# ducha-aiki/mods-light-zmq

Hardware: AMD Instinct MI355X
Metric: image_pairs_per_sec_end_to_end (higher is better)
Workload: dtype f32

## Files before the change

### include/mods_hip.h

```cpp
#ifndef MODS_HIP_H
#define MODS_HIP_H

#include <stddef.h>
#include <stdint.h>

#ifdef __cplusplus
extern "C" {
#endif

#define MODS_OK 0
#define MODS_E_NODEVICE (-1)
#define MODS_E_ARG (-2)
#define MODS_E_CAPACITY (-3)
#define MODS_E_HIP (-4)

typedef struct mods_ctx mods_ctx;

typedef struct mods_hessaff_params {
  int numberOfScales;
  float initialSigma;
  float threshold;
  float edgeEigenValueRatio;
  int border;
  int maxIterations;
// ... 68 lines not shown
       MODS_STAGE_LOCAL_AFFINE,
       MODS_STAGE_COUNT };
int mods_ctx_timing_enable(mods_ctx *ctx, int stage_mask);
int mods_ctx_graphs(mods_ctx *ctx, int on);
long mods_ctx_graph_replays(const mods_ctx *ctx);
long mods_ctx_u8_source_calls(const mods_ctx *ctx);
int mods_ctx_u8_kernels(mods_ctx *ctx, int mask);
long mods_ctx_u8_strip_calls(const mods_ctx *ctx);
int mods_u8_strips_layout(int w, int h, unsigned *max_width, unsigned *n_strips, unsigned *pitch, size_t *image_bytes);
void mods_u8_strips_strip_of(unsigned n, unsigned *out);
int mods_u8_strips_offsets(int w, int h, unsigned *out);
int mods_u8_strips_fetch(mods_ctx *ctx, const unsigned char *img_u8_host, int n_img, int w, int h, int src_offset, unsigned char *out);
int mods_ctx_pyramid_streams(mods_ctx *ctx, int n);
int mods_ctx_timing_read(mods_ctx *ctx, int stage, double *total_ms, int *launches, double *bytes);
int mods_ctx_timing_reset(mods_ctx *ctx);

int mods_detect_hessian_affine(mods_ctx *ctx, const float *img, int w, int h, int stride,
                               const mods_hessaff_params *par, mods_affkey *out, int max_out, int *n_out);
int mods_detect_hessian_affine_dev(mods_ctx *ctx, const float *img_dev, int n_img, int w, int h, int stride,
                                   const mods_hessaff_params *par, mods_affkey *out_host, int max_out,
                                   int *n_out_host);

int mods_pyramid_octaves(mods_ctx *ctx);
int mods_pyramid_dims(mods_ctx *ctx, int octave, int *w, int *h);
int mods_pyramid_plane(mods_ctx *ctx, int img, int octave, int level, int kind, float *dst_host);
int mods_pyramid_candidates(mods_ctx *ctx, int img, mods_candidate *out, int max_out, int *n_out);
int mods_pyramid_nms_hits(mods_ctx *ctx, int img, int *out4, int max_out, int *n_out);

int mods_gauss_blur(mods_ctx *ctx, const float *src, int w, int h, float sigma, float *dst);
int mods_hessian_response(mods_ctx *ctx, const float *src, int w, int h, float norm, float *dst);
int mods_resize_half(mods_ctx *ctx, const float *src, int w, int h, float *dst, int *dw, int *dh);

typedef struct mods_describe_params {
  double ori_mrSize;
  int ori_patchSize;
  int ori_maxAngles;
  double ori_threshold;
  double desc_mrSize;
  int desc_patchSize;
  int photoNorm;
  int rootSift;
  double maxBinValue;
  int ori_halfMode;
  int addUpRight;
  int halfDesc;
  int fastExtraction;
} mods_describe_params;

int mods_orient_describe(mods_ctx *ctx, const float *img, int w, int h, int stride, const mods_affkey *keys,
                         int n_keys, const mods_describe_params *par, mods_region *out, int max_out, int *n_out);

int mods_orient_describe_u8(mods_ctx *ctx, const unsigned char *img_u8, int w, int h, int stride, const mods_affkey *keys,
                            int n_keys, const mods_describe_params *par, mods_region *out, int max_out, int *n_out);

int mods_detect_describe_dev(mods_ctx *ctx, const float *img_dev, int n_img, int w, int h, int stride,
                             const mods_hessaff_params *det, const mods_describe_params *desc,
                             int *n_detected_host, int *n_regions_host);
int mods_detect_describe_dev_u8(mods_ctx *ctx, const unsigned char *img_u8_dev, int n_img, int w, int h, int stride,
                                const mods_hessaff_params *det, const mods_describe_params *desc,
                                int *n_detected_host, int *n_regions_host);
typedef int (*mods_descriptor_fn)(void *user, const float *patches, int n, int ps, float *out, size_t out_cap_floats, int *dim);
int mods_ctx_set_external_descriptor(mods_ctx *ctx, mods_descriptor_fn fn, void *user, double mrSize, int patchSize);
int mods_ctx_set_external_shape(mods_ctx *ctx, mods_descriptor_fn fn, void *user, double mrSize, int patchSize);
int mods_ctx_set_external_orientation(mods_ctx *ctx, mods_descriptor_fn fn, void *user, double mrSize, int patchSize);
typedef struct mods_net mods_net;
enum { MODS_NET_AFFNET = 0, MODS_NET_ORINET = 1, MODS_NET_HARDNET = 2 };
int  mods_net_create(int device, int kind, const float *const *tensors, const size_t *n_floats, int n_tensors, mods_net **out);
void mods_net_destroy(mods_net *net);
int  mods_net_dim(const mods_net *net);
int  mods_net_chunk(void);
int  mods_net_forward(mods_net *net, const float *patches_host, int n, int quantise_u8, float *out_host);
int  mods_net_forward_dev(mods_net *net, void *hip_stream, const float *patches_dev, int n, int quantise_u8, float *out_dev);
int  mods_ctx_set_builtin_shape(mods_ctx *ctx, mods_net *net, double mrSize, int quantise_u8);
int  mods_ctx_set_builtin_orientation(mods_ctx *ctx, mods_net *net, double mrSize, int quantise_u8);
int  mods_ctx_set_builtin_descriptor(mods_ctx *ctx, mods_net *net, double mrSize, int quantise_u8);
int  mods_test_net_stage(mods_net *net, int stage, const float *in_host, int n, int quantise_u8, float *out_host, int *guard_ok);
int mods_patches_fetch(mods_ctx *ctx, int img, int ps, float *out, int max_regions, int *n_out);
int mods_baumberg_stats_enable(mods_ctx *ctx, int on);
int mods_baumberg_stats(mods_ctx *ctx, int img, unsigned long long *keypoints, unsigned long long *iterations);
int mods_unoriented_count(mods_ctx *ctx, int img);
int mods_regions_fetch(mods_ctx *ctx, int img, mods_region *out, int max_out, int *n_out);

int mods_dominant_angle(mods_ctx *ctx, const float *patch, int ps, double th, float *angle, int *found);
int mods_selftest_fast_sqrt(mods_ctx *ctx, unsigned long long *out5);
int mods_sift_patch(mods_ctx *ctx, const float *patch, int ps, int rootsift, double maxBinValue, uint8_t *out128);

typedef struct mods_view_geom {
  int identity;
  int w_rot, h_rot;
  int w_new, h_new;
  int ksize_x, ksize_y, pad;
  double rotation, tilt, zoom;
  double sigma_x, sigma_y;
  double H[9];
  double warpRot[6], warpTilt[6];
} mods_view_geom;

int mods_view_geometry(int w, int h, double tilt, double phi, double zoom, double initSigma, mods_view_geom *out);
int mods_synth_view_dev(mods_ctx *ctx, const float *src_dev, int w, int h, int stride, const mods_view_geom *geom, int doBlur,
                        float *dst_dev);
int mods_detect_describe_view_dev(mods_ctx *ctx, const float *src_dev, int w, int h, int stride, double tilt, double phi,
                                  double zoom, double initSigma, int doBlur, const mods_hessaff_params *det,
                                  const mods_describe_params *desc, mods_view_geom *geom_out, int *n_detected, int *n_regions);
int mods_detect_describe_view2_dev(mods_ctx *ctx, const float *src1_dev, const float *src2_dev, int w, int h, int stride, double tilt,
                                   double phi, double zoom, double initSigma, int doBlur, const mods_hessaff_params *det,
                                   const mods_describe_params *desc, mods_view_geom *geom_out, int *n_detected2, int *n_regions2);
const mods_region *mods_regions_dev(mods_ctx *ctx, int img);
const mods_region *mods_regions_half_dev(mods_ctx *ctx, int img);
int mods_regions_fetch_half(mods_ctx *ctx, int img, mods_region *out, int max_out, int *n_out);
int mods_regions_copy_dev(mods_ctx *ctx, int img, mods_region *dst_dev, int n);
const float *mods_view_pixels_dev(mods_ctx *ctx);
int mods_view_fetch(mods_ctx *ctx, const mods_view_geom *geom, float *dst_host);
int mods_warp_affine(mods_ctx *ctx, const float *src, int w, int h, const double *M, int dw, int dh, float cval, float *dst);
int mods_gauss_blur_xy(mods_ctx *ctx, const float *src, int w, int h, int kx, int ky, double sx, double sy, float *dst);

int mods_match_fginn(mods_ctx *ctx, const mods_region *q, int n_q, const mods_region *t, int n_t, double ratio,
                     double contradDist, int nn, mods_tentative *out, double *u6_out, double *laf_out, int max_out, int *n_out);
int mods_match_distance(mods_ctx *ctx, const mods_region *q, int n_q, const mods_region *t, int n_t, double threshold,
                        mods_tentative *out, double *u6_out, double *laf_out, int max_out, int *n_out);
int mods_match_dev(mods_ctx *ctx, int img_q, int img_t, double ratio, double contradDist, int nn, mods_tentative *out,
                   double *u6_out, double *laf_out, int max_out, int *n_out);
int mods_match_grid(int n_q, int n_t, int out[3]);

int mods_duplicate_filter(mods_tentative *tent, double *u6, double *laf, int n, double r, int mode, int *n_out);
int mods_duplicate_filter_gpu(mods_ctx *ctx, mods_tentative *tent, double *u6, double *laf, int n, double r, int mode, int *n_out,
                              int *on_device);

typedef struct mods_ransac_params {
  double err_threshold;
  double confidence;
  int max_samples;
  int localOptimization;
  double LAFCoef;
  double HLAFCoef;
  int errorType;
  int doSymmCheck;
  int useF;
  int groundTruth;
  int ransacForStopping;
  double gtH[9];
} mods_ransac_params;

int mods_hmatrix_filter(const double *u6, int n, const double *H_rowmajor, const mods_ransac_params *par, unsigned char *mask, int *n_true);

int mods_loransac_h(const double *u6, const double *laf, int n, const mods_ransac_params *par, unsigned char *mask,
                    double *H_out, int *n_inliers, int *stats3);
int mods_loransac_f(const double *u6, const double *laf, int n, const mods_ransac_params *par, unsigned char *mask,
                    double *F_out, int *n_inliers, int *stats3);
int mods_orsa_f(const double *u6, const double *laf, int n, int w, int h, const mods_ransac_params *par, unsigned char *mask,
                double *F_out, int *n_inliers, float *log_nfa, int *index_out, int *n_index, int *stats3);
int mods_orsa_f_ex(const double *u6, const double *laf, int n, int w, int h, const mods_ransac_params *par, unsigned char *mask,
                   double *F_out, int *n_inliers, float *log_nfa, int *index_out, int *n_index, int *stats3, int on_device, int batch,
                   int wg_keys);
int mods_orsa_last_profile(double *ms5, long *launches);
int mods_test_orsa_epipolar(const float *p1, const float *p2, const int *k7, float *F1, float *F2, float *z);
int mods_test_orsa_tables(int n, float *logcn, float *logc7);
int mods_test_orsa_log10(const float *x, int n, float *out);
int mods_test_orsa_score(const float *p1, const float *p2, int n, int w, int h, const float *F, int m, int on_device, int wg_keys,
                         int *out4);
long long mods_test_orsa_log10_sweep(unsigned begin, unsigned count, unsigned *list, int max_list);
struct mods_pair_params;
int mods_verify_tentatives(int device, const struct mods_pair_params *par, mods_tentative *tent, double *u6, double *laf, int n,
                           int *n_unique, int *n_verified, double *H_out, int *stats3, double *ms_dup, double *ms_ransac);
int mods_verify_tentatives_ex(int device, const struct mods_pair_params *par, mods_tentative *tent, double *u6, double *laf, int n,
                              int *n_unique, int *n_verified, double *H_out, int *stats3, int *gt3, double *ms_dup, double *ms_ransac);
int mods_verify_tentatives_wh(int device, const struct mods_pair_params *par, mods_tentative *tent, double *u6, double *laf, int n,
// ... 275 lines not shown
```

### mods-light-zmq_amd/csrc/capi.hip

```cpp
#include "common.hpp"
#include "u8_strips.hpp"
#include "detmath.hpp"
#include "ransac_host.hpp"
#include "f_laf.hpp"
#include "../../include/mods_degensac.h"
#include <cstdarg>
#include <memory>
#include <algorithm>
#include <cmath>
#include <mutex>
#include <vector>
#include <time.h>
#include <sys/prctl.h>

namespace mods {

static thread_local char g_err[512] = "";

void set_error(const char *fmt, ...) {
  va_list ap;
  va_start(ap, fmt);
  vsnprintf(g_err, sizeof(g_err), fmt, ap);
  va_end(ap);
}

template <class T> struct HandlePool {
  std::mutex mu;
  std::vector<T> free_[16];
  T take(int dev, T (*make)()) {
    { std::lock_guard<std::mutex> lk(mu); if (!free_[dev].empty()) { T h = free_[dev].back(); free_[dev].pop_back(); return h; } }
    return make();
  }
  void give(int dev, T h) { std::lock_guard<std::mutex> lk(mu); free_[dev].push_back(h); }
};
template <class T> struct Borrowed {
  HandlePool<T> *pool; T h[16] = {};
  explicit Borrowed(HandlePool<T> *p) : pool(p) {}
  ~Borrowed() { for (int d = 0; d < 16; d++) if (h[d]) pool->give(d, h[d]); }
};
static HandlePool<hipEvent_t> *event_pool() { static HandlePool<hipEvent_t> *p = new HandlePool<hipEvent_t>(); return p; }
static HandlePool<hipStream_t> *stream_pool() { static HandlePool<hipStream_t> *p = new HandlePool<hipStream_t>(); return p; }
static hipEvent_t thread_event(hipStream_t s) {
  static thread_local Borrowed<hipEvent_t> t(event_pool());
  int cur = 0, dev = 0;
  if (hipGetDevice(&cur) != hipSuccess) return nullptr;
  dev = cur;
  if (s && hipStreamGetDevice(s, &dev) != hipSuccess) { (void)hipGetLastError(); return nullptr; }
  if (dev < 0 || dev >= 16) return nullptr;
  if (!t.h[dev]) {
    if (dev != cur && hipSetDevice(dev) != hipSuccess) { (void)hipGetLastError(); return nullptr; }
    t.h[dev] = t.pool->take(dev, +[]() -> hipEvent_t { hipEvent_t e = nullptr; return hipEventCreateWithFlags(&e, hipEventDisableTiming) == hipSuccess ? e : nullptr; });
    if (dev != cur) (void)hipSetDevice(cur);
  }
  return t.h[dev];
}
hipError_t stream_wait(hipStream_t s) {
  const long ns = tl_wait_sleep_ns;
  if (ns <= 0) return hipStreamSynchronize(s);
  hipEvent_t ev = thread_event(s);
  if (!ev) return hipStreamSynchronize(s);
  hipError_t e = hipEventRecord(ev, s);
  if (e != hipSuccess) { (void)hipGetLastError(); return hipStreamSynchronize(s); }
  e = hipEventQuery(ev);
  for (int i = 0; i < tl_wait_spin_polls && e == hipErrorNotReady; i++) e = hipEventQuery(ev);
  long cur = ns;
  const long cap = std::max(ns, tl_wait_sleep_max_ns);
  while (e == hipErrorNotReady) {
    const timespec ts = {0, cur};
    nanosleep(&ts, nullptr);
    e = hipEventQuery(ev);
    cur = std::min(cap, cur + cur / 2);
  }
  const hipError_t last = hipGetLastError();
  if (e == hipSuccess && last != hipSuccess && last != hipErrorNotReady) return last;
  return e;
}

static bool capturing(hipStream_t s) {
  hipStreamCaptureStatus st = hipStreamCaptureStatusNone;
  if (hipStreamIsCapturing(s, &st) != hipSuccess) { (void)hipGetLastError(); return false; }
  return st != hipStreamCaptureStatusNone;
}
hipError_t copy_wait(hipStream_t s, void *dst, const void *src, size_t bytes, hipMemcpyKind kind) {
// ... 536 lines not shown
  if (!c || img < 0 || img >= c->batch || !n_out) return MODS_E_ARG;
  MODS_HIP_CHECK(hipSetDevice(c->device));
  MODS_HIP_CHECK(mods::stream_wait(c->stream));
  int n = 0;
  MODS_HIP_CHECK(mods::copy_wait(c->stream, &n, c->region_count + img, sizeof(int), hipMemcpyDeviceToHost));
  *n_out = n;
  if (out) {
    if (n > max_out) { set_error("region output overflow: %d > %d", n, max_out); return MODS_E_CAPACITY; }
    MODS_HIP_CHECK(mods::copy_wait(c->stream, out, c->regions_dev + (size_t)img * c->max_cand, sizeof(mods_region) * n, hipMemcpyDeviceToHost));
  }
  return MODS_OK;
}

int mods_regions_fetch_half(mods_ctx *c, int img, mods_region *out, int max_out, int *n_out) {
  if (!c || img < 0 || img >= c->batch || !n_out) return MODS_E_ARG;
  if (!c->have_half || !c->regions_half_dev) { set_error("no HalfRootSIFT descriptors: the last describe call did not ask for them"); return MODS_E_ARG; }
  MODS_HIP_CHECK(hipSetDevice(c->device));
  MODS_HIP_CHECK(mods::stream_wait(c->stream));
  int n = 0;
  MODS_HIP_CHECK(mods::copy_wait(c->stream, &n, c->region_count + img, sizeof(int), hipMemcpyDeviceToHost));
  *n_out = n;
  if (out) {
    if (n > max_out) { set_error("region output overflow: %d > %d", n, max_out); return MODS_E_CAPACITY; }
    MODS_HIP_CHECK(mods::copy_wait(c->stream, out, c->regions_half_dev + (size_t)img * c->max_cand, sizeof(mods_region) * n, hipMemcpyDeviceToHost));
  }
  return MODS_OK;
}
const mods_region *mods_regions_half_dev(mods_ctx *c, int img) {
  return (c && c->have_half && c->regions_half_dev) ? c->regions_half_dev + (size_t)img * c->max_cand : nullptr;
}

int mods_orient_describe(mods_ctx *c, const float *img, int w, int h, int stride, const mods_affkey *keys, int n_keys,
                         const mods_describe_params *par, mods_region *out, int max_out, int *n_out) {
  if (!c || !img || !par || !n_out || (n_keys > 0 && !keys)) { set_error("orient_describe: null argument"); return MODS_E_ARG; }
  if ((size_t)w * h > (size_t)c->max_w * c->max_h) { set_error("image larger than the context"); return MODS_E_ARG; }
  if (n_keys > c->max_cand) { set_error("too many keypoints for the context: %d > %d", n_keys, c->max_cand); return MODS_E_CAPACITY; }
  MODS_HIP_CHECK(hipSetDevice(c->device));
  MODS_HIP_CHECK(hipMemcpy2DAsync(c->input_dev, sizeof(float) * w, img, sizeof(float) * stride, sizeof(float) * w, h,
                                  hipMemcpyHostToDevice, c->stream));
  MODS_HIP_CHECK(hipMemcpyAsync(c->keys_dev, keys, sizeof(mods_affkey) * n_keys, hipMemcpyHostToDevice, c->stream));
  MODS_HIP_CHECK(hipMemcpyAsync(c->cand_count + 2 * c->batch, &n_keys, sizeof(int), hipMemcpyHostToDevice, c->stream));
  MODS_HIP_CHECK(mods::stream_wait(c->stream));
  int rc = describe_run(c, {c->input_dev}, 1, w, h, par);
  if (rc) return rc;
  if ((rc = mods_regions_fetch(c, 0, out, max_out, n_out))) return rc;
  return check_desc_err(c);
}

int mods_orient_describe_u8(mods_ctx *c, const unsigned char *img_u8, int w, int h, int stride, const mods_affkey *keys, int n_keys,
                            const mods_describe_params *par, mods_region *out, int max_out, int *n_out) {
  if (!img_u8 || !par || !n_out || (n_keys > 0 && !keys)) { set_error("orient_describe_u8: null argument"); return MODS_E_ARG; }
  if (w < 1 || h < 1) { set_error("orient_describe_u8: image size %d x %d", w, h); return MODS_E_ARG; }
  if (stride < w) { set_error("orient_describe_u8: stride %d < width %d", stride, w); return MODS_E_ARG; }
  if (n_keys < 0) { set_error("orient_describe_u8: %d keypoints", n_keys); return MODS_E_ARG; }
  if (!c) { set_error("orient_describe_u8: null context"); return MODS_E_ARG; }
  if ((size_t)w * h > (size_t)c->max_w * c->max_h) { set_error("orient_describe_u8: image %d x %d larger than the context", w, h); return MODS_E_ARG; }
  if (n_keys > c->max_cand) { set_error("orient_describe_u8: too many keypoints for the context: %d > %d", n_keys, c->max_cand); return MODS_E_ARG; }
  MODS_HIP_CHECK(hipSetDevice(c->device));
  int rc;
  if ((rc = mods::u8_stage_ensure(c))) return rc;
  MODS_HIP_CHECK(hipMemcpy2DAsync(c->u8_stage_dev, w, img_u8, stride, w, h, hipMemcpyHostToDevice, c->stream));
  MODS_HIP_CHECK(hipMemcpyAsync(c->keys_dev, keys, sizeof(mods_affkey) * n_keys, hipMemcpyHostToDevice, c->stream));
  MODS_HIP_CHECK(hipMemcpyAsync(c->cand_count + 2 * c->batch, &n_keys, sizeof(int), hipMemcpyHostToDevice, c->stream));
  MODS_HIP_CHECK(mods::stream_wait(c->stream));
  PixelSources img;
  if ((rc = mods::u8_sources_launch(c, c->u8_stage_dev, 1, w, h, w, true, &img))) return rc;
  if ((rc = describe_run(c, img, 1, w, h, par))) return rc;
  if ((rc = mods_regions_fetch(c, 0, out, max_out, n_out))) return rc;
  return check_desc_err(c);
}

int mods_dominant_angle(mods_ctx *c, const float *patch, int ps, double th, float *angle, int *found) {
  mods_describe_params dp = {5.1962, ps, 1, th, 5.1962, c->desc_ps ? c->desc_ps : 41, 1, 1, 0.2};
  MODS_HIP_CHECK(hipSetDevice(c->device));
  int rc = describe_configure(c, &dp);
  if (rc) return rc;
  MODS_HIP_CHECK(hipMemcpyAsync(c->input_dev, patch, sizeof(float) * ps * ps, hipMemcpyHostToDevice, c->stream));
  if ((rc = launch_dominant_angle_test(c, c->input_dev, ps, th, c->tmp_dev))) return rc;
  float res[2];
  MODS_HIP_CHECK(hipMemcpyAsync(res, c->tmp_dev, sizeof(res), hipMemcpyDeviceToHost, c->stream));
  MODS_HIP_CHECK(mods::stream_wait(c->stream));
  *found = res[0] != 0.f;
  *angle = res[1];
  return MODS_OK;
}

int mods_selftest_fast_sqrt(mods_ctx *c, unsigned long long *out5) {
  if (!c || !out5) { set_error("selftest: null argument"); return MODS_E_ARG; }
  MODS_HIP_CHECK(hipSetDevice(c->device));
  return launch_fast_sqrt_selftest(c, out5);
}

int mods_sift_patch(mods_ctx *c, const float *patch, int ps, int rootsift, double maxBinValue, uint8_t *out128) {
  mods_describe_params dp = {5.1962, c->desc_ori_ps ? c->desc_ori_ps : 32, 1, 0.8, 5.1962, ps, 1, rootsift, maxBinValue};
  MODS_HIP_CHECK(hipSetDevice(c->device));
  int rc = describe_configure(c, &dp);
  if (rc) return rc;
  MODS_HIP_CHECK(hipMemcpyAsync(c->input_dev, patch, sizeof(float) * ps * ps, hipMemcpyHostToDevice, c->stream));
  if ((rc = launch_sift_patch_test(c, c->input_dev, ps, rootsift, maxBinValue, (uint8_t *)c->tmp_dev.get()))) return rc;
  MODS_HIP_CHECK(hipMemcpyAsync(out128, c->tmp_dev, 128, hipMemcpyDeviceToHost, c->stream));
  MODS_HIP_CHECK(mods::stream_wait(c->stream));
  return MODS_OK;
}

static int dsp_args(const char *who, int K, double a, double b) {
  if (K == 0 || K == 1) return MODS_OK;
  if (K < 0 || K > 8) { set_error("%s: numScales %d (0 or 1: off; 2 .. 8)", who, K); return MODS_E_ARG; }
  if (!std::isfinite(a) || !(a > 0)) { set_error("%s: startCoef %g (finite, > 0)", who, a); return MODS_E_ARG; }
  if (!std::isfinite(b) || !(b > a) || b > 4) { set_error("%s: endCoef %g (finite, startCoef < endCoef <= 4)", who, b); return MODS_E_ARG; }
  return MODS_OK;
}
int mods_ctx_domain_pooling(mods_ctx *c, int numScales, double startCoef, double endCoef) {
  const int rc = dsp_args("domain_pooling", numScales, startCoef, endCoef);
  if (rc) return rc;
  if (!c) { set_error("domain_pooling: null context"); return MODS_E_ARG; }
  const bool on = numScales >= 2;
  c->dsp_scales = on ? numScales : 0;
  c->dsp_start = on ? startCoef : 0;
  c->dsp_end = on ? endCoef : 0;
  mods::dev_state_changed(c);
  return MODS_OK;
}
int mods_ctx_domain_pooling_get(const mods_ctx *c, int *numScales, double *startCoef, double *endCoef) {
  if (!c) { set_error("domain_pooling_get: null context"); return MODS_E_ARG; }
  if (numScales) *numScales = c->dsp_scales;
  if (startCoef) *startCoef = c->dsp_start;
  if (endCoef) *endCoef = c->dsp_end;
  return MODS_OK;
}
int mods_test_sift_pooled(mods_ctx *c, const float *patches, int K, int ps, int rootsift, int half, int photoNorm, double maxBinValue,
                          uint8_t *out128) {
  if (!c || !patches || !out128) { set_error("test_sift_pooled: null argument"); return MODS_E_ARG; }
  if (K < 1 || K > 8) { set_error("test_sift_pooled: %d patches (1 .. 8)", K); return MODS_E_ARG; }
  if ((size_t)K * ps * ps > (size_t)c->max_w * c->max_h * c->batch) { set_error("test_sift_pooled: the patches do not fit the context's input buffer"); return MODS_E_ARG; }
  mods_describe_params dp = {5.1962, c->desc_ori_ps ? c->desc_ori_ps : 32, 1, 0.8, 5.1962, ps, photoNorm, rootsift, maxBinValue};
  MODS_HIP_CHECK(hipSetDevice(c->device));
  int rc = describe_configure(c, &dp);
  if (rc) return rc;
  MODS_HIP_CHECK(hipMemcpyAsync(c->input_dev, patches, sizeof(float) * (size_t)K * ps * ps, hipMemcpyHostToDevice, c->stream));
  if ((rc = launch_sift_pooled_test(c, c->input_dev, K, ps, rootsift, half, photoNorm, maxBinValue, (uint8_t *)c->tmp_dev.get()))) return rc;
  MODS_HIP_CHECK(hipMemcpyAsync(out128, c->tmp_dev, 128, hipMemcpyDeviceToHost, c->stream));
  MODS_HIP_CHECK(mods::stream_wait(c->stream));
  return MODS_OK;
}

int mods_match_copy_out(mods_ctx *c, int n, mods_tentative *tent, double *u6, double *laf) {
  if (n <= 0) return MODS_OK;
  static thread_local std::vector<char> stage;
  stage.resize(tent_bytes((size_t)n));
  MODS_HIP_CHECK(hipMemcpyAsync(stage.data(), c->m_tent, stage.size(), hipMemcpyDeviceToHost, c->stream));
  MODS_HIP_CHECK(mods::stream_wait(c->stream));
  tent_unpack(stage.data(), (size_t)n, tent, u6, laf);
  return MODS_OK;
}

int mods_match_fetch_internal(mods_ctx *c, mods_tentative *out, double *u6_out, double *laf_out, int max_out, int *n_out) {
  MODS_HIP_CHECK(mods::stream_wait(c->stream));
  const int n = read_slot(c->m_count, count_slot());
  *n_out = n;
  if (n > max_out) { set_error("tentative output overflow: %d > %d", n, max_out); return MODS_E_CAPACITY; }
  return mods_match_copy_out(c, n, out, u6_out, laf_out);
}

static int match_upload(mods_ctx *c, const mods_region *q, int n_q, const mods_region *t, int n_t, const int *n_out) {
  if (!c || !n_out || (n_q > 0 && !q) || (n_t > 0 && !t)) { set_error("match: null argument"); return MODS_E_ARG; }
  MODS_HIP_CHECK(hipSetDevice(c->device));
// ... 403 lines not shown
```

### mods-light-zmq_amd/csrc/describe_common.hpp

```cpp
#pragma once
#include "common.hpp"

namespace mods {

struct DescConst {
  int w, h;
  int max_cand, max_reg;
  int reg_cap;
  double ks;
  int ori_ps;
  double ori_i2p;
  int max_angles;
  int ori_cap;
  double ori_th;
  int ori_half;
  int add_upright;
  int half_desc;
  double desc_mr;
  int desc_ps;
  int photo, root;
  double max_bin;
  int p2_lo, p2_hi;
  size_t scratch_stride;
  int tap_cap;
  int patch_rule;
  int view;
  int ow, oh;
  double Hinv[6];
};

struct SiftTab {
  int bin0[64], bin1[64];
  float w0[64], w1[64];
};

int launch_extract_and_sift(mods_ctx *ctx, const PixelSources &img, int n_img, DescConst k, const float *dmask, const SiftTab *tab,
                            bool run_sift = true);
int launch_half_sift(mods_ctx *ctx, int n_img, DescConst k, const float *dmask, const SiftTab *tab);
int launch_sift_patch_test(mods_ctx *ctx, const float *patch_dev, int ps, int root, double max_bin, uint8_t *out_dev);
int launch_dsp_accumulate(mods_ctx *ctx, int n_img, DescConst k, const float *dmask, const SiftTab *tab, bool first);
int launch_dsp_finish(mods_ctx *ctx, int n_img, DescConst k, bool want_half);

}
```

### mods-light-zmq_amd/csrc/device_util.hpp

```cpp
#pragma once
#include <hip/hip_runtime.h>
#include <type_traits>
#include "atan_lut_data.h"
#include "u8_strips.hpp"

namespace mods {

__host__ __device__ __forceinline__ bool check_borders(int img_w, int img_h, float ofsx, float ofsy, float a11, float a12,
                                              float a21, float a22, int res_w, int res_h) {
  const int width = img_w - 2, height = img_h - 2;
  const float halfWidth = (float)ceil((double)((float)res_w) / 2.0);
  const float halfHeight = (float)ceil((double)((float)res_h) / 2.0);
  const float xs[4] = {-halfWidth, -halfWidth, +halfWidth, +halfWidth};
  const float ys[4] = {-halfHeight, +halfHeight, -halfHeight, +halfHeight};
  bool touch = false;
#pragma unroll
  for (int i = 0; i < 4; i++) {
    float imx = ofsx + xs[i] * a11 + ys[i] * a12;
    float imy = ofsy + xs[i] * a21 + ys[i] * a22;
    if (floorf(imx) <= 0 || floorf(imy) <= 0 || ceilf(imx) >= width || ceilf(imy) >= height) touch = true;
  }
  return touch;
}

template <class T> __device__ __forceinline__ T *as_global(T *p) {
  typedef __attribute__((address_space(1))) T GT;
  GT *g = (GT *)(unsigned long long)p;
  return (T *)g;
}

__device__ __forceinline__ float lane_up1(float x) {
  return __int_as_float(__builtin_amdgcn_update_dpp(__float_as_int(x), __float_as_int(x), 0x138, 0xf, 0xf, false));
}
__device__ __forceinline__ float lane_down1(float x) {
  return __int_as_float(__builtin_amdgcn_update_dpp(__float_as_int(x), __float_as_int(x), 0x130, 0xf, 0xf, false));
}
__device__ __forceinline__ void wave_sync() {
  __builtin_amdgcn_fence(__ATOMIC_RELEASE, "wavefront");
  __builtin_amdgcn_wave_barrier();
  __builtin_amdgcn_fence(__ATOMIC_ACQUIRE, "wavefront");
}

__device__ __forceinline__ float fast_sqrtf(float x) {
  float s = __builtin_amdgcn_sqrtf(x);
  const float sd = __int_as_float(__float_as_int(s) - 1), su = __int_as_float(__float_as_int(s) + 1);
  const float vp = fmaf(-sd, s, x), vs = fmaf(-su, s, x);
  s = vp <= 0.f ? sd : s;
  s = vs > 0.f ? su : s;
  return s;
}
__device__ __forceinline__ float fast_sqrtf_any(float x) {
  const bool tiny = (unsigned)(__float_as_int(x) - 1) < (unsigned)(0x0f800000 - 1);
  if (__builtin_expect(__builtin_amdgcn_ballot_w64(tiny) != 0ull, 0)) return sqrtf(x);
  return fast_sqrtf(x);
}

struct __attribute__((packed, aligned(4))) PixPair { float a, b; };
struct __attribute__((packed, aligned(1))) PixPairU8 { unsigned char a, b; };
__device__ __forceinline__ void pix_pair(const float *__restrict__ p, float &a, float &b) { const PixPair q = *(const PixPair *)p; a = q.a; b = q.b; }
__device__ __forceinline__ void pix_pair(const unsigned char *__restrict__ p, float &a, float &b) {
  const PixPairU8 q = *(const PixPairU8 *)p;
  a = (float)q.a; b = (float)q.b;
}
struct StripPx { unsigned char v; };
__device__ __forceinline__ void pix_pair(const StripPx *__restrict__ p, float &a, float &b) { pix_pair((const unsigned char *)p, a, b); }
template <class PX> constexpr bool kStripSource = std::is_same<PX, StripPx>::value;
template <class PX> __device__ __forceinline__ const PX *batch_image(const PX *__restrict__ all, int w, int h, int b) {
  if constexpr (kStripSource<PX>) return all + strip_image_bytes(w, h) * b;
  else return all + (size_t)w * h * b;
}
template <class PX> __device__ __forceinline__ unsigned pix_index(int w, int h, int x, int y) {
  if constexpr (kStripSource<PX>) return strip_offset((unsigned)x, (unsigned)y, strip_pitch(h));
  else return (unsigned)(__mul24(y, w) + x);
}
template <class PX> __device__ __forceinline__ int pix_row_step(int w) { return kStripSource<PX> ? kStripRowBytes : w; }

struct TapLoads { float r00, r01, r10, r11, wx, wy; bool valid; };
template <class PX>
__device__ __forceinline__ TapLoads tap_load(const PX *__restrict__ im, int w, int h, float WX, float WY, bool touch) {
  TapLoads t;
  int x, y;
  if (!touch) { x = (int)WX; y = (int)WY; t.valid = true; }
  else { x = (int)floorf(WX); y = (int)floorf(WY); t.valid = WX >= 0 && WY >= 0 && x < w - 1 && y < h - 1; }
  t.wx = WX - (float)x;
  t.wy = WY - (float)y;
  if (t.valid) {
    const PX *Row0 = kStripSource<PX> ? im + pix_index<PX>(w, h, x, y) : im + (size_t)y * w + x;
    pix_pair(Row0, t.r00, t.r01); pix_pair(Row0 + pix_row_step<PX>(w), t.r10, t.r11);
  } else { t.r00 = t.r01 = t.r10 = t.r11 = 0.f; }
  return t;
}
template <class PX>
__device__ __forceinline__ TapLoads tap_load_bf(const PX *__restrict__ im, int w, int h, float WX, float WY, bool touch) {
  TapLoads t;
  const int x = (int)floorf(WX), y = (int)floorf(WY);
  t.valid = !touch || (WX >= 0 && WY >= 0 && x < w - 1 && y < h - 1);
  t.wx = WX - (float)x;
  t.wy = WY - (float)y;
  const int xc = min(max(x, 0), w - 2), yc = min(max(y, 0), h - 2);
  const PX *Row0 = im + pix_index<PX>(w, h, xc, yc);
  pix_pair(Row0, t.r00, t.r01); pix_pair(Row0 + pix_row_step<PX>(w), t.r10, t.r11);
  return t;
}
__device__ __forceinline__ float tap_combine(const TapLoads &t) {
  if (!t.valid) return 0.f;
  const float I1 = t.wx * (t.r01 - t.r00) + t.r00;
  return t.wy * (t.wx * (t.r11 - t.r10) + t.r10 - I1) + I1;
}

template <class PX>
__device__ __forceinline__ TapLoads tap_load_inside(const PX *__restrict__ im, int w, int h, float WX, float WY, bool inwin) {
  TapLoads t;
  const int x = (int)WX, y = (int)WY;
  t.valid = true;
  t.wx = WX - (float)x;
  t.wy = WY - (float)y;
  const PX *Row0 = im + (inwin ? pix_index<PX>(w, h, x, y) : 0u);
  pix_pair(Row0, t.r00, t.r01); pix_pair(Row0 + pix_row_step<PX>(w), t.r10, t.r11);
// ... 148 lines not shown
```

### mods-light-zmq_amd/csrc/sift.hip

```cpp
#include "describe_common.hpp"
#include "detmath.hpp"
#include "device_util.hpp"

namespace mods {

constexpr int SMALL_CAP = 80;
#ifndef EXTRACT_T_LO
#define EXTRACT_T_LO 48
#endif
#ifndef EXTRACT_T_MID
#define EXTRACT_T_MID 64
#endif
#ifndef ES_MINB
#define ES_MINB 5
#endif

__device__ __forceinline__ double *lds_doubles(float *base, const void *p) {
  const int off = (int)((const float *)p - base);
  return (double *)(base + ((off + 1) & ~1));
}

struct RegionGeom {
  int P2;
  float scale;
// ... 992 lines not shown
__global__ __launch_bounds__(256, 5) void sift_kernel(DescConst k, const float *__restrict__ patches, mods_region *__restrict__ reg_all,
                                                   const int *__restrict__ reg_count, const float *__restrict__ mask,
                                                   const SiftTab *__restrict__ tab) {
  extern __shared__ __attribute__((aligned(16))) float smem[];
  const int ps = k.desc_ps, pp = ps * ps;
  SiftLds L(smem, ps);
  const int tid = threadIdx.x;
  const int b = blockIdx.y;
  const int n_mask = sift_block_setup(L, mask, tab, ps);
  mods_region *reg = reg_all + (size_t)b * k.max_reg;
  int n = reg_count[b];
  if (n > k.reg_cap) n = k.reg_cap;
  for (int ri = blockIdx.x; ri < n; ri += gridDim.x) {
    const float *src = patches + ((size_t)b * k.reg_cap + ri) * pp;
    __syncthreads();
    for (int p = tid; p < pp; p += 256) L.patch[p] = src[p];
    __syncthreads();
    if (k.photo) photonorm_patch(L.patch, L.midx, n_mask, L.g, pp, L.redf);
    sift_from_patch(L.patch, mask, L.w, L.lut, ps, k.root != 0, k.max_bin, L.px, L.bo, L.vec, L.red, reg[ri].desc, k.half_desc != 0);
  }
}

__global__ __launch_bounds__(256, 5) void dsp_accumulate_kernel(DescConst k, const float *__restrict__ patches, double *__restrict__ acc,
                                                                const int *__restrict__ reg_count, const float *__restrict__ mask,
                                                                const SiftTab *__restrict__ tab, int first) {
  extern __shared__ __attribute__((aligned(16))) float smem[];
  const int ps = k.desc_ps, pp = ps * ps;
  SiftLds L(smem, ps);
  const int tid = threadIdx.x;
  const int b = blockIdx.y;
  const int n_mask = sift_block_setup(L, mask, tab, ps);
  int n = reg_count[b];
  if (n > k.reg_cap) n = k.reg_cap;
  for (int ri = blockIdx.x; ri < n; ri += gridDim.x) {
    const size_t slot = (size_t)b * k.reg_cap + ri;
    const float *src = patches + slot * pp;
    __syncthreads();
    for (int p = tid; p < pp; p += 256) L.patch[p] = src[p];
    __syncthreads();
    if (k.photo) photonorm_patch(L.patch, L.midx, n_mask, L.g, pp, L.redf);
    sift_hist_from_patch(L.patch, mask, L.w, L.lut, ps, L.px, L.bo, L.vec);
    if (tid < 128) {
      double *a = acc + slot * 128;
      a[tid] = first ? L.vec[tid] : a[tid] + L.vec[tid];
    }
  }
}

__global__ __launch_bounds__(128) void dsp_finish_kernel(DescConst k, const double *__restrict__ acc, const int *__restrict__ reg_count,
                                                         uint8_t *__restrict__ out, uint8_t *__restrict__ out_half, size_t img_stride,
                                                         size_t reg_stride) {
  __shared__ double s_vec[128], s_sq[128], s_red[2];
  const int tid = threadIdx.x;
  const int b = blockIdx.y;
  int n = reg_count[b];
  if (n > k.reg_cap) n = k.reg_cap;
  for (int ri = blockIdx.x; ri < n; ri += gridDim.x) {
    const double *a = acc + ((size_t)b * k.reg_cap + ri) * 128;
    for (int half = 0; half < 2; half++) {
      uint8_t *o = half ? out_half : out;
      if (!o) continue;
      s_vec[tid] = a[tid];
      __syncthreads();
      sift_tail(s_vec, s_sq, s_red, k.root != 0, k.max_bin, o + (size_t)b * img_stride + (size_t)ri * reg_stride, half != 0);
    }
  }
}

constexpr int SW_R = 8;
constexpr int SW_G = 68;
constexpr int SW_CW = 18;
constexpr int S2_MAX_IMG = 64;
constexpr int S2_WAVES = 12;
constexpr int S2_BINS = 1024;
__device__ __forceinline__ int s2_bin(int g, int br, int bc) { return (g >> 2) * 64 + br * 16 + (g & 3) * 4 + bc; }
__device__ __forceinline__ int s2_vec(int g, int i) { return (i & 7) * 128 + s2_bin(g, i >> 5, (i >> 3) & 3); }

__host__ __device__ constexpr int s2_row_slots(int ps) { return SW_R * ps + SW_CW + 2 > SW_R * SW_G / 2 ? SW_R * ps + SW_CW + 2 : SW_R * SW_G / 2; }
static size_t sift_wave2_wave_bytes(int ps) {
  return sizeof(double) * S2_BINS + sizeof(float2) * (size_t)s2_row_slots(ps) + sizeof(float) * 3 * SW_R;
}
static size_t sift_wave2_lds_bytes(int ps) {
  const size_t ppa = ((size_t)ps * ps + 7) & ~(size_t)7;
  return sizeof(float) * 2048 + sizeof(float) * (4 * ps + 4) + sizeof(int) * 72 + sizeof(unsigned short) * ppa + S2_WAVES * sift_wave2_wave_bytes(ps) + 64;
}

template <int NC, bool POOL = false>
__global__ __launch_bounds__(64 * S2_WAVES, 3) void sift_wave2_kernel(DescConst k, const float *__restrict__ patches, mods_region *__restrict__ reg_all,
                                                                        const int *__restrict__ reg_count, const float *__restrict__ mask,
                                                                        const SiftTab *__restrict__ tab, int n_img, int *__restrict__ next_unit,
                                                                        double *__restrict__ pool, int pool_first) {
  extern __shared__ __attribute__((aligned(16))) float smem[];
  const int ps = k.desc_ps, pp = ps * ps, ppa = (pp + 7) & ~7;
  const int tid = threadIdx.x, lane = tid & 63, wv = tid >> 6;
  float *s_ot = smem;
  float *s_w = s_ot + 2048;
  int *s_pref = (int *)(s_w + 4 * ps + 4);
  unsigned short *s_midx = (unsigned short *)(s_pref + 72);
  unsigned char *wbase = (unsigned char *)(s_midx + ppa) + (size_t)wv * (sizeof(double) * S2_BINS + sizeof(float2) * s2_row_slots(ps) + sizeof(float) * 3 * SW_R);
  double *acc = (double *)wbase;
  float2 *pxrow = (float2 *)(acc + S2_BINS);
  float *s_mean = (float *)(pxrow + s2_row_slots(ps)), *s_fac = s_mean + SW_R;
  int *s_flag = (int *)(s_fac + SW_R);
  float *g = (float *)pxrow;
  const int rowf = SW_R * ps;

  const double M_PI_DOUBLED = 6.28318530718;
  sift_tables(tab, ps, s_w);
  for (int i = tid; i < 2048; i += 64 * S2_WAVES) {
    const float ori = atan2_lut_case(i >> 8, g_atan_lut[i & 255]);
    s_ot[i] = (float)(8.0f * ((double)ori + M_PI_DOUBLED) / M_PI_DOUBLED);
  }
  if (tid < 64) {
    int c = 0;
    for (int base = 0; base < pp; base += 64) {
      const int p = base + tid;
      const bool m = p < pp && mask[p] > 0;
      const unsigned long long bm = __ballot(m);
      if (m) s_midx[c + __popcll(bm & ((1ull << tid) - 1ull))] = (unsigned short)p;
      c += __popcll(bm);
    }
    if (tid == 0) s_pref[68] = c;
  }
  if (tid == 64) {
    int cum = 0;
    for (int b = 0; b < n_img; b++) { s_pref[b] = cum; int n = reg_count[b]; if (n > k.reg_cap) n = k.reg_cap; cum += (n + SW_R - 1) / SW_R; }
    s_pref[n_img] = cum;
  }
  __syncthreads();
  const int n_mask = s_pref[68];
  const int total_units = s_pref[n_img];
  const float o_zero = (float)(8.0f * ((double)0.f + M_PI_DOUBLED) / M_PI_DOUBLED);

  const int hr = lane >> 3, hsel = (lane >> 2) & 1, hbc = lane & 3;
  int clo = ps;
  for (int i = ps - 1; i >= 0; i--) if (s_w[hbc * ps + i] > 0) clo = i;
  float wcw[NC];
#pragma unroll
  for (int q = 0; q < NC; q++) wcw[q] = (clo + q < ps) ? s_w[hbc * ps + clo + q] : 0.f;
  constexpr int RL = 6;
  int s_rr[RL], s_c[RL];
#pragma unroll
  for (int u = 0; u < RL; u++) { const int e = lane + 64 * u; s_rr[u] = e < rowf ? e / ps : SW_R - 1; s_c[u] = e < rowf ? e - (e / ps) * ps : 0; }

#ifdef SIFT_PROF
  unsigned long long pt[6] = {0, 0, 0, 0, 0, 0}, pl = __builtin_amdgcn_s_memtime();
  int pn = 0;
#define S2PROF(i) { const unsigned long long t_ = __builtin_amdgcn_s_memtime(); pt[i] += t_ - pl; pl = t_; }
#else
#define S2PROF(i)
#endif
  for (;;) {
    int unit = 0;
    if (lane == 0) unit = atomicAdd(next_unit, 1);
    unit = __builtin_amdgcn_readfirstlane(unit);
    if (unit >= total_units) break;
    int b = 0;
    while (b + 1 < n_img && s_pref[b + 1] <= unit) b++;
    const int ri0 = (unit - s_pref[b]) * SW_R;
    mods_region *reg = reg_all + (size_t)b * k.max_reg;
    int n = reg_count[b];
    if (n > k.reg_cap) n = k.reg_cap;
    const float *pbase = patches + (size_t)b * k.reg_cap * pp;
    auto patch_of = [&](int rr) { return pbase + (size_t)min(ri0 + rr, n - 1) * pp; };
    wave_sync();
    S2PROF(0)
#pragma unroll
    for (int i = 0; i < S2_BINS / 64; i++) acc[lane + 64 * i] = 0.0;
    if (lane < SW_R) { s_flag[lane] = 0; s_mean[lane] = 0.f; s_fac[lane] = 0.f; }
    if (k.photo) {
      for (int pass = 0; pass < 2; pass++) {
        float sum = 0.f;
        float v[SW_R];
        {
          const int idx = s_midx[min(lane, n_mask - 1)];
#pragma unroll
          for (int rr = 0; rr < SW_R; rr++) v[rr] = patch_of(rr)[idx];
        }
        for (int q0 = 0; q0 < n_mask; q0 += 64) {
          const int cnt = min(64, n_mask - q0);
          wave_sync();
#pragma unroll
          for (int rr = 0; rr < SW_R; rr++) {
            float x = v[rr];
            if (pass) { const float d = s_mean[rr] - x; x = d * d; }
            g[rr * SW_G + lane] = x;
          }
          if (q0 + 64 < n_mask) {
            const int idx = s_midx[min(q0 + 64 + lane, n_mask - 1)];
#pragma unroll
            for (int rr = 0; rr < SW_R; rr++) v[rr] = patch_of(rr)[idx];
          }
          wave_sync();
          if (lane < SW_R) {
            const float *gl = g + lane * SW_G;
            int q = 0;
            for (; q + 15 < cnt; q += 16) {
              const float4 a0 = *(const float4 *)(gl + q), a1 = *(const float4 *)(gl + q + 4), a2 = *(const float4 *)(gl + q + 8), a3 = *(const float4 *)(gl + q + 12);
              sum += a0.x; sum += a0.y; sum += a0.z; sum += a0.w; sum += a1.x; sum += a1.y; sum += a1.z; sum += a1.w;
              sum += a2.x; sum += a2.y; sum += a2.z; sum += a2.w; sum += a3.x; sum += a3.y; sum += a3.z; sum += a3.w;
            }
            for (; q + 3 < cnt; q += 4) {
              const float4 a = *(const float4 *)(gl + q);
              sum += a.x; sum += a.y; sum += a.z; sum += a.w;
            }
            for (; q < cnt; q++) sum += gl[q];
          }
        }
        if (lane < SW_R) {
          if (pass == 0) s_mean[lane] = sum / (float)n_mask;
          else {
            const float var = sqrtf(sum / (float)n_mask);
            if (!((double)var < 0.0001)) { s_flag[lane] = 1; s_fac[lane] = 50.0f / var; }
          }
        }
        wave_sync();
      }
    }
    wave_sync();
    S2PROF(1)
    unsigned sbyte[RL], cbyte[RL];
    float sm[RL], sf[RL];
    unsigned nflag = 0;
#pragma unroll
    for (int u = 0; u < RL; u++) {
      sbyte[u] = ((unsigned)min(ri0 + s_rr[u], n - 1) * (unsigned)pp + (unsigned)s_c[u]) * 4u;
      cbyte[u] = (unsigned)s_c[u] * 4u;
      sm[u] = s_mean[s_rr[u]]; sf[u] = s_fac[s_rr[u]];
      nflag |= (s_flag[s_rr[u]] ? 1u : 0u) << u;
    }
    auto fetch_row = [&](int r, float *dst) {
      const char *rowp = (const char *)(pbase + r * ps);
#pragma unroll
      for (int u = 0; u < RL; u++) dst[u] = *(const float *)(rowp + sbyte[u]);
    };
    auto norm_row = [&](const float *raw, float *dst) {
#pragma unroll
      for (int u = 0; u < RL; u++) {
        const float t = __builtin_amdgcn_fmed3f(128 + sf[u] * (raw[u] - sm[u]), 0.f, 255.f);
        dst[u] = ((nflag >> u) & 1) ? t : raw[u];
      }
    };
    auto fetch_mask = [&](int r, float *dst) {
      const char *mrowp = (const char *)(mask + r * ps);
#pragma unroll
      for (int u = 0; u < RL; u++) dst[u] = *(const float *)(mrowp + cbyte[u]);
    };
    float nm[RL], n0[RL], np[RL], ra[RL], rb[RL], mcur[RL];
    fetch_row(0, ra); norm_row(ra, n0);
    fetch_row(min(1, ps - 1), ra); norm_row(ra, np);
    fetch_row(min(2, ps - 1), ra);
    fetch_row(min(3, ps - 1), rb);
    fetch_mask(0, mcur);
#pragma unroll
    for (int u = 0; u < RL; u++) nm[u] = n0[u];
#pragma unroll 1
    for (int r = 0; r < ps; r++) {
      {
        const unsigned last_col = 4u * (unsigned)(ps - 1);
#pragma unroll
        for (int u = 0; u < RL; u++) {
          const int e = lane + 64 * u;
          float right = lane_down1(n0[u]), left = lane_up1(n0[u]);
          if (u + 1 < RL) { const float nx = __int_as_float(__builtin_amdgcn_readlane(__float_as_int(n0[u + 1 < RL ? u + 1 : u]), 0)); right = lane == 63 ? nx : right; }
          if (u > 0) { const float pl = __int_as_float(__builtin_amdgcn_readlane(__float_as_int(n0[u > 0 ? u - 1 : u]), 63)); left = lane == 0 ? pl : left; }
          const float xa = cbyte[u] < last_col ? right : n0[u];
          const float xb = cbyte[u] > 0u ? left : n0[u];
          const float xgrad = xa - xb, ygrad = np[u] - nm[u];
          const float grad = fast_sqrtf_any(xgrad * xgrad + ygrad * ygrad);
          const AtanSel as = atan2_lut_sel(ygrad, xgrad);
          const float ot = s_ot[as.oct * 256 + as.idx];
          const float o = as.zero ? o_zero : ot;
          if (e < rowf) pxrow[e] = make_float2(mcur[u] * grad, o);
        }
      }
      fetch_mask(min(r + 1, ps - 1), mcur);
      wave_sync();
      S2PROF(2)
      {
        const int rb8 = hsel ? tab->bin1[r] : tab->bin0[r];
        const float wrr = hsel ? tab->w1[r] : tab->w0[r];
        if (wrr > 0) {
          double *abin = acc + s2_bin(hr, rb8 >> 3, hbc);
          const float2 *px = pxrow + hr * ps + clo;
#pragma unroll
          for (int q0 = 0; q0 < NC; q0 += NC / 2) {
            float2 pv[NC / 2];
#pragma unroll
            for (int q = 0; q < NC / 2; q++) pv[q] = px[q0 + q];
#pragma unroll
            for (int q = 0; q < NC / 2; q++) {
              const float val = wrr * (wcw[q0 + q] * pv[q].x);
              const bool on = val > 0;
              const int bo0 = (int)pv[q].y;
              const float y = pv[q].y - bo0;
              const float c0 = on ? val * (1.0f - y) : 0.f, c1 = on ? val * y : 0.f;
              __hip_atomic_fetch_add(abin + (bo0 & 7) * 128, (double)c0, __ATOMIC_RELAXED, __HIP_MEMORY_SCOPE_WAVEFRONT);
              __hip_atomic_fetch_add(abin + ((bo0 + 1) & 7) * 128, (double)c1, __ATOMIC_RELAXED, __HIP_MEMORY_SCOPE_WAVEFRONT);
            }
          }
        }
      }
      wave_sync();
      S2PROF(3)
#pragma unroll
      for (int u = 0; u < RL; u++) { nm[u] = n0[u]; n0[u] = np[u]; }
      norm_row(ra, np);
#pragma unroll
      for (int u = 0; u < RL; u++) ra[u] = rb[u];
      fetch_row(min(r + 4, ps - 1), rb);
      S2PROF(4)
    }
    wave_sync();
    if constexpr (POOL) {
      const int rr = lane >> 3;
      if (ri0 + rr < n) {
        double *dst = pool + ((size_t)b * k.reg_cap + ri0 + rr) * 128;
        for (int i = lane & 7; i < 128; i += 8) {
          const double x = acc[s2_vec(rr, i)];
          dst[i] = pool_first ? x : dst[i] + x;
        }
      }
      continue;
    }
    double *tmp = (double *)pxrow;
    unsigned long long redo = ~0ull;
    for (int pass = 0; pass < 2; pass++) {
      if (lane < SW_R && ((redo >> (8 * lane)) & 1)) {
        double len = 0.0;
#pragma unroll 1
        for (int i = 0; i < 128; i += 8) {
          double x[8];
#pragma unroll
          for (int q = 0; q < 8; q++) x[q] = acc[s2_vec(lane, i + q)];
#pragma unroll
          for (int q = 0; q < 8; q++) x[q] = x[q] * x[q];
          len += x[0] + x[1] + x[2] + x[3];
          len += x[4] + x[5] + x[6] + x[7];
        }
        len = sqrt(len);
        tmp[lane] = 1.0 / len;
      }
      wave_sync();
      bool changed = false;
      {
        const int rr = lane >> 3;
        if ((redo >> (8 * rr)) & 1) {
          const double inv = tmp[rr];
          for (int i = lane & 7; i < 128; i += 8) {
            double *vp = acc + s2_vec(rr, i);
            double x = *vp * inv;
            if (pass == 0 && x > k.max_bin) { x = k.max_bin; changed = true; }
            *vp = x;
          }
        }
      }
      const unsigned long long ch = __ballot(changed);
      unsigned long long next = 0;
      for (int rr = 0; rr < SW_R; rr++)
        if ((ch >> (8 * rr)) & 0xffull) next |= 0xffull << (8 * rr);
      redo = next;
      wave_sync();
      if (!redo) break;
    }
    if (k.root) {
      if (lane < SW_R) {
        double sum = 0.;
#pragma unroll 1
        for (int i = 0; i < 128; i += 8) {
          double x[8];
#pragma unroll
          for (int q = 0; q < 8; q++) x[q] = acc[s2_vec(lane, i + q)];
#pragma unroll
          for (int q = 0; q < 8; q++) sum += fabs(x[q]);
        }
        tmp[lane] = sum;
      }
      wave_sync();
    }
    {
      const int rr = lane >> 3;
      if (ri0 + rr < n) {
        const double rs = k.root ? tmp[rr] : 1.0;
        uint32_t *out = (uint32_t *)reg[ri0 + rr].desc;
        for (int w4 = lane & 7; w4 < 32; w4 += 8) {
          uint32_t word = 0;
// ... 232 lines not shown
```

Baseline: 1069.

## Remap SIFT wave lanes to 8-column groups and skip masked-out row spans

Changes the per-lane pixel mapping in the wave SIFT kernel so each lane handles a fixed region row with columns strided by 8, replacing cross-lane shuffles and per-element mean/factor lookups with DPP row shifts and scalar per-lane values. Precomputes per-row nonzero spans of the circular Gaussian mask in LDS and skips gradient/orientation computation for column groups and whole rows outside the mask, zeroing stale pixel slots only when needed. Adds a host test entry point for the span computation. Risks correctness if the lane remapping or dirty-slot tracking mishandles edge columns, and adds a small amount of LDS.

After: 1075 (median of 4 runs). No clear change (+0.6%).

```diff
diff --git a/include/mods_hip.h b/include/mods_hip.h
--- a/include/mods_hip.h
+++ b/include/mods_hip.h
@@ -174,6 +174,7 @@
 int mods_regions_fetch(mods_ctx *ctx, int img, mods_region *out, int max_out, int *n_out);
 
 int mods_dominant_angle(mods_ctx *ctx, const float *patch, int ps, double th, float *angle, int *found);
+int mods_test_mask_spans(int size, float sigma, int *lo, int *hi);
 int mods_selftest_fast_sqrt(mods_ctx *ctx, unsigned long long *out5);
 int mods_sift_patch(mods_ctx *ctx, const float *patch, int ps, int rootsift, double maxBinValue, uint8_t *out128);
 
diff --git a/mods-light-zmq_amd/csrc/capi.hip b/mods-light-zmq_amd/csrc/capi.hip
--- a/mods-light-zmq_amd/csrc/capi.hip
+++ b/mods-light-zmq_amd/csrc/capi.hip
@@ -1,4 +1,5 @@
 #include "common.hpp"
+#include "describe_common.hpp"
 #include "u8_strips.hpp"
 #include "detmath.hpp"
 #include "ransac_host.hpp"
@@ -701,6 +702,14 @@
   MODS_HIP_CHECK(mods::stream_wait(c->stream));
   *found = res[0] != 0.f;
   *angle = res[1];
+  return MODS_OK;
+}
+
+int mods_test_mask_spans(int size, float sigma, int *lo, int *hi) {
+  if (size < 1 || size > 64 || !lo || !hi) { set_error("test_mask_spans: size %d (1 .. 64) or null argument", size); return MODS_E_ARG; }
+  std::vector<float> m((size_t)64 * 64, 0.f);
+  circular_gauss_mask_host(size, sigma, m.data());
+  for (int r = 0; r < size; r++) mods::mask_row_span(m.data(), size, r, lo + r, hi + r);
   return MODS_OK;
 }
 
diff --git a/mods-light-zmq_amd/csrc/describe_common.hpp b/mods-light-zmq_amd/csrc/describe_common.hpp
--- a/mods-light-zmq_amd/csrc/describe_common.hpp
+++ b/mods-light-zmq_amd/csrc/describe_common.hpp
@@ -34,6 +34,13 @@
   float w0[64], w1[64];
 };
 
+__host__ __device__ inline void mask_row_span(const float *mask, int size, int r, int *lo, int *hi) {
+  int l = size, h = -1;
+  for (int c = 0; c < size; c++)
+    if (mask[r * size + c] > 0) { if (l == size) l = c; h = c; }
+  *lo = l; *hi = h;
+}
+
 int launch_extract_and_sift(mods_ctx *ctx, const PixelSources &img, int n_img, DescConst k, const float *dmask, const SiftTab *tab,
                             bool run_sift = true);
 int launch_half_sift(mods_ctx *ctx, int n_img, DescConst k, const float *dmask, const SiftTab *tab);
diff --git a/mods-light-zmq_amd/csrc/device_util.hpp b/mods-light-zmq_amd/csrc/device_util.hpp
--- a/mods-light-zmq_amd/csrc/device_util.hpp
+++ b/mods-light-zmq_amd/csrc/device_util.hpp
@@ -34,6 +34,12 @@
 }
 __device__ __forceinline__ float lane_down1(float x) {
   return __int_as_float(__builtin_amdgcn_update_dpp(__float_as_int(x), __float_as_int(x), 0x130, 0xf, 0xf, false));
+}
+template <int D> __device__ __forceinline__ float row_up(float x) {
+  return __int_as_float(__builtin_amdgcn_update_dpp(__float_as_int(x), __float_as_int(x), 0x110 + D, 0xf, 0xf, false));
+}
+template <int D> __device__ __forceinline__ float row_down(float x) {
+  return __int_as_float(__builtin_amdgcn_update_dpp(__float_as_int(x), __float_as_int(x), 0x100 + D, 0xf, 0xf, false));
 }
 __device__ __forceinline__ void wave_sync() {
   __builtin_amdgcn_fence(__ATOMIC_RELEASE, "wavefront");
diff --git a/mods-light-zmq_amd/csrc/sift.hip b/mods-light-zmq_amd/csrc/sift.hip
--- a/mods-light-zmq_amd/csrc/sift.hip
+++ b/mods-light-zmq_amd/csrc/sift.hip
@@ -1098,7 +1098,7 @@
 }
 static size_t sift_wave2_lds_bytes(int ps) {
   const size_t ppa = ((size_t)ps * ps + 7) & ~(size_t)7;
-  return sizeof(float) * 2048 + sizeof(float) * (4 * ps + 4) + sizeof(int) * 72 + sizeof(unsigned short) * ppa + S2_WAVES * sift_wave2_wave_bytes(ps) + 64;
+  return sizeof(float) * 2048 + sizeof(float) * (4 * ps + 4) + sizeof(int) * 72 + sizeof(unsigned short) * (ppa + 64) + S2_WAVES * sift_wave2_wave_bytes(ps) + 64;
 }
 
 template <int NC, bool POOL = false>
@@ -1113,13 +1113,13 @@
   float *s_w = s_ot + 2048;
   int *s_pref = (int *)(s_w + 4 * ps + 4);
   unsigned short *s_midx = (unsigned short *)(s_pref + 72);
-  unsigned char *wbase = (unsigned char *)(s_midx + ppa) + (size_t)wv * (sizeof(double) * S2_BINS + sizeof(float2) * s2_row_slots(ps) + sizeof(float) * 3 * SW_R);
+  unsigned short *s_span = s_midx + ppa;
+  unsigned char *wbase = (unsigned char *)(s_span + 64) + (size_t)wv * (sizeof(double) * S2_BINS + sizeof(float2) * s2_row_slots(ps) + sizeof(float) * 3 * SW_R);
   double *acc = (double *)wbase;
   float2 *pxrow = (float2 *)(acc + S2_BINS);
   float *s_mean = (float *)(pxrow + s2_row_slots(ps)), *s_fac = s_mean + SW_R;
   int *s_flag = (int *)(s_fac + SW_R);
   float *g = (float *)pxrow;
-  const int rowf = SW_R * ps;
 
   const double M_PI_DOUBLED = 6.28318530718;
   sift_tables(tab, ps, s_w);
@@ -1143,6 +1143,11 @@
     for (int b = 0; b < n_img; b++) { s_pref[b] = cum; int n = reg_count[b]; if (n > k.reg_cap) n = k.reg_cap; cum += (n + SW_R - 1) / SW_R; }
     s_pref[n_img] = cum;
   }
+  if (tid >= 128 && tid < 128 + ps) {
+    int lo, hi;
+    mask_row_span(mask, ps, tid - 128, &lo, &hi);
+    s_span[tid - 128] = hi < 0 ? (unsigned short)255 : (unsigned short)(lo | (hi << 8));
+  }
   __syncthreads();
   const int n_mask = s_pref[68];
   const int total_units = s_pref[n_img];
@@ -1155,9 +1160,7 @@
 #pragma unroll
   for (int q = 0; q < NC; q++) wcw[q] = (clo + q < ps) ? s_w[hbc * ps + clo + q] : 0.f;
   constexpr int RL = 6;
-  int s_rr[RL], s_c[RL];
-#pragma unroll
-  for (int u = 0; u < RL; u++) { const int e = lane + 64 * u; s_rr[u] = e < rowf ? e / ps : SW_R - 1; s_c[u] = e < rowf ? e - (e / ps) * ps : 0; }
+  const int prr = lane >> 3, cib = lane & 7;
 
 #ifdef SIFT_PROF
   unsigned long long pt[6] = {0, 0, 0, 0, 0, 0}, pl = __builtin_amdgcn_s_memtime();
@@ -1236,14 +1239,12 @@
     wave_sync();
     S2PROF(1)
     unsigned sbyte[RL], cbyte[RL];
-    float sm[RL], sf[RL];
-    unsigned nflag = 0;
+    const float sm = s_mean[prr], sf = s_fac[prr];
+    const bool nflag = s_flag[prr] != 0;
 #pragma unroll
     for (int u = 0; u < RL; u++) {
-      sbyte[u] = ((unsigned)min(ri0 + s_rr[u], n - 1) * (unsigned)pp + (unsigned)s_c[u]) * 4u;
-      cbyte[u] = (unsigned)s_c[u] * 4u;
-      sm[u] = s_mean[s_rr[u]]; sf[u] = s_fac[s_rr[u]];
-      nflag |= (s_flag[s_rr[u]] ? 1u : 0u) << u;
+      cbyte[u] = (unsigned)min(8 * u + cib, ps - 1) * 4u;
+      sbyte[u] = (unsigned)min(ri0 + prr, n - 1) * (unsigned)pp * 4u + cbyte[u];
     }
     auto fetch_row = [&](int r, float *dst) {
       const char *rowp = (const char *)(pbase + r * ps);
@@ -1253,8 +1254,8 @@
     auto norm_row = [&](const float *raw, float *dst) {
 #pragma unroll
       for (int u = 0; u < RL; u++) {
-        const float t = __builtin_amdgcn_fmed3f(128 + sf[u] * (raw[u] - sm[u]), 0.f, 255.f);
-        dst[u] = ((nflag >> u) & 1) ? t : raw[u];
+        const float t = __builtin_amdgcn_fmed3f(128 + sf * (raw[u] - sm), 0.f, 255.f);
+        dst[u] = nflag ? t : raw[u];
       }
     };
     auto fetch_mask = [&](int r, float *dst) {
@@ -1270,24 +1271,35 @@
     fetch_mask(0, mcur);
 #pragma unroll
     for (int u = 0; u < RL; u++) nm[u] = n0[u];
+    unsigned dirty = (1u << RL) - 1;
 #pragma unroll 1
     for (int r = 0; r < ps; r++) {
+      const int span = __builtin_amdgcn_readfirstlane((int)s_span[r]);
+      const int span_lo = span & 255, span_hi = span >> 8;
+      if (span_lo <= span_hi) {
       {
         const unsigned last_col = 4u * (unsigned)(ps - 1);
 #pragma unroll
         for (int u = 0; u < RL; u++) {
-          const int e = lane + 64 * u;
-          float right = lane_down1(n0[u]), left = lane_up1(n0[u]);
-          if (u + 1 < RL) { const float nx = __int_as_float(__builtin_amdgcn_readlane(__float_as_int(n0[u + 1 < RL ? u + 1 : u]), 0)); right = lane == 63 ? nx : right; }
-          if (u > 0) { const float pl = __int_as_float(__builtin_amdgcn_readlane(__float_as_int(n0[u > 0 ? u - 1 : u]), 63)); left = lane == 0 ? pl : left; }
-          const float xa = cbyte[u] < last_col ? right : n0[u];
-          const float xb = cbyte[u] > 0u ? left : n0[u];
-          const float xgrad = xa - xb, ygrad = np[u] - nm[u];
-          const float grad = fast_sqrtf_any(xgrad * xgrad + ygrad * ygrad);
-          const AtanSel as = atan2_lut_sel(ygrad, xgrad);
-          const float ot = s_ot[as.oct * 256 + as.idx];
-          const float o = as.zero ? o_zero : ot;
-          if (e < rowf) pxrow[e] = make_float2(mcur[u] * grad, o);
+          const bool stores = 8 * u + cib < ps;
+          float2 *pxe = pxrow + prr * ps + 8 * u + cib;
+          if (8 * u <= span_hi && 8 * u + 7 >= span_lo) {
+            float right = row_down<1>(n0[u]), left = row_up<1>(n0[u]);
+            if (u + 1 < RL) { const float nx = row_up<7>(n0[u + 1 < RL ? u + 1 : u]); right = cib == 7 ? nx : right; }
+            if (u > 0) { const float pl = row_down<7>(n0[u > 0 ? u - 1 : u]); left = cib == 0 ? pl : left; }
+            const float xa = cbyte[u] < last_col ? right : n0[u];
+            const float xb = cbyte[u] > 0u ? left : n0[u];
+            const float xgrad = xa - xb, ygrad = np[u] - nm[u];
+            const float grad = fast_sqrtf_any(xgrad * xgrad + ygrad * ygrad);
+            const AtanSel as = atan2_lut_sel(ygrad, xgrad);
+            const float ot = s_ot[as.oct * 256 + as.idx];
+            const float o = as.zero ? o_zero : ot;
+            if (stores) *pxe = make_float2(mcur[u] * grad, o);
+            dirty |= 1u << u;
+          } else if ((dirty >> u) & 1) {
+            if (stores) *pxe = make_float2(0.f, o_zero);
+            dirty &= ~(1u << u);
+          }
         }
       }
       fetch_mask(min(r + 1, ps - 1), mcur);
@@ -1318,6 +1330,7 @@
         }
       }
       wave_sync();
+      } else fetch_mask(min(r + 1, ps - 1), mcur);
       S2PROF(3)
 #pragma unroll
       for (int u = 0; u < RL; u++) { nm[u] = n0[u]; n0[u] = np[u]; }
```
